# Chairy-neko/TinyRayTracing

Hardware: AMD Instinct MI355X
Metric: Mrays/s (higher is better)
Workload: dtype f32

## Files before the change

tinyraytracing_amd/csrc/trt_api.hip:

```cpp
#include <hip/hip_runtime.h>

#include <dlfcn.h>

#include <algorithm>
#include <cstdio>
#include <cstdlib>
#include <atomic>
#include <limits>
#include <chrono>
#include <cstring>
#include <condition_variable>
#include <memory>
#include <mutex>
#include <string>
#include <thread>
#include <vector>

#include "trt.h"
#include "trt_kernels.h"
#include "trt_wide.h"
#include "trt_oct_build.h"

using namespace trtd;

// ... 50 lines not shown

struct trt_handle {
    int device = 0;
    SceneDev sc{};
    std::vector<void*> scene_allocs;
    std::vector<uint32_t> light_mats;
    std::vector<LightBox> light_boxes;
    uint32_t depth = 0;
    uint32_t bvh2_depth = 0;
    uint32_t shade_tabs = 0;
    uint32_t shade_pad_lds = 0;
    const void* lds_image = nullptr;
    uint32_t lds_image_bytes = 0;
    uint32_t lds_tab[5] = {0, 0, 0, 0, 0};
    int trace_impl = 3;
    int node_kind = 0;
    uint32_t oct_levels = 0;
    bool dbg = false;
    uint32_t rays_per_wave = 256, fill_blocks = 2048, max_blocks = 8192;
    uint32_t traceGrid(uint32_t n) const
    {
        uint32_t b = (n + TRT_TRACE_BLOCK - 1) / TRT_TRACE_BLOCK;
        if (rays_per_wave > 64) {
            const uint32_t want = (uint32_t)(((uint64_t)n + 4ull * rays_per_wave - 1) / (4ull * rays_per_wave));
            b = std::min(b, std::max(fill_blocks, want));
        }
        b = std::min(std::max(b, 8u), std::min(max_blocks, 8192u));
        return (b + 7u) & ~7u;
    }
    uint32_t tail_n = 131072;
// ... 182 lines not shown
        end(stream);
        st.launches[k]++;
    }
};

using ClosestKernel = void (*)(SceneDev, RaySource, f4*, uint32_t, uint32_t*, uint32_t, DeviceStats*, RedoList);
using ShadowKernel = void (*)(SceneDev, ShadowQueue, uint32_t, uint32_t, f4*, uint32_t*, uint32_t, DeviceStats*, uint32_t, RedoList, LightBox);
using FixKernel = void (*)(SceneDev, RaySource, f4*, const f4*, uint32_t, f4*, uint32_t*, uint32_t, RedoList, uint32_t, DeviceStats*);
using ShadeKernel = void (*)(SceneDev, ShadeArgs);
using TailKernel = void (*)(SceneDev, TailArgs);

constexpr uint32_t OCT_LDS_LEVELS = 10;
int traversalOf(const trt_handle* h) { return h->trace_impl == 0 ? 0 : (h->node_kind == 1 ? 1 : (h->depth <= 16 ? 2 : 3)); }
ClosestKernel closestKernel(const trt_handle* h, bool count, int primary)
{
    const ClosestKernel k[4][2][3] = {
        {{k_trace_closest<false, 1, false, 0, 0, 0>, k_trace_closest<false, 1, false, 0, 1, 0>, k_trace_closest<false, 1, false, 0, PRIMARY_LIST, 0>},
         {k_trace_closest<true, 1, false, 0, 0, 0>, k_trace_closest<true, 1, false, 0, 1, 0>, k_trace_closest<true, 1, false, 0, PRIMARY_LIST, 0>}},
        {{k_trace_closest<false, OCT_LDS_LEVELS, true, 3, 0, 1>, k_trace_closest<false, OCT_LDS_LEVELS, true, 3, 1, 1>, k_trace_closest<false, OCT_LDS_LEVELS, true, 3, PRIMARY_LIST, 1>},
         {k_trace_closest<true, OCT_LDS_LEVELS, true, 3, 0, 1>, k_trace_closest<true, OCT_LDS_LEVELS, true, 3, 1, 1>, k_trace_closest<true, OCT_LDS_LEVELS, true, 3, PRIMARY_LIST, 1>}},
        {{k_trace_closest<false, 16, false, 3, 0, 0>, k_trace_closest<false, 16, false, 3, 1, 0>, k_trace_closest<false, 16, false, 3, PRIMARY_LIST, 0>},
         {k_trace_closest<true, 16, false, 3, 0, 0>, k_trace_closest<true, 16, false, 3, 1, 0>, k_trace_closest<true, 16, false, 3, PRIMARY_LIST, 0>}},
        {{k_trace_closest<false, TRT_LDS_STACK_MAX, true, 3, 0, 0>, k_trace_closest<false, TRT_LDS_STACK_MAX, true, 3, 1, 0>, k_trace_closest<false, TRT_LDS_STACK_MAX, true, 3, PRIMARY_LIST, 0>},
         {k_trace_closest<true, TRT_LDS_STACK_MAX, true, 3, 0, 0>, k_trace_closest<true, TRT_LDS_STACK_MAX, true, 3, 1, 0>, k_trace_closest<true, TRT_LDS_STACK_MAX, true, 3, PRIMARY_LIST, 0>}}};
    return k[traversalOf(h)][count][primary];
}
ShadowKernel shadowKernel(const trt_handle* h, bool count)
{
    const ShadowKernel k[4][2] = {{k_trace_shadow<false, 1, false, 0, 0>, k_trace_shadow<true, 1, false, 0, 0>},
                                  {k_trace_shadow<false, OCT_LDS_LEVELS, true, 3, 1>, k_trace_shadow<true, OCT_LDS_LEVELS, true, 3, 1>},
                                  {k_trace_shadow<false, 16, false, 3, 0>, k_trace_shadow<true, 16, false, 3, 0>},
                                  {k_trace_shadow<false, TRT_LDS_STACK_MAX, true, 3, 0>, k_trace_shadow<true, TRT_LDS_STACK_MAX, true, 3, 0>}};
    return k[traversalOf(h)][count];
}
FixKernel fixKernel(const trt_handle* h, bool shadow, int primary)
{
    const FixKernel k[4] = {k_trace_fix<false, 0, 0>, k_trace_fix<false, 1, 0>, k_trace_fix<false, PRIMARY_LIST, 0>, k_trace_fix<true, false, 0>};
    return h->trace_impl == 0 ? nullptr : k[shadow ? 3 : primary];
}
ShadeKernel shadeKernel(uint32_t tabs, int lights, bool list)
{
    const ShadeKernel k[5][2][3] = {
        {{k_shade<31u, SHADE_ONE>, k_shade<31u, SHADE_FEW>, k_shade<31u, SHADE_MANY>}, {k_shade<31u, SHADE_ONE, true>, k_shade<31u, SHADE_FEW, true>, k_shade<31u, SHADE_MANY, true>}},
        {{k_shade<15u, SHADE_ONE>, k_shade<15u, SHADE_FEW>, k_shade<15u, SHADE_MANY>}, {k_shade<15u, SHADE_ONE, true>, k_shade<15u, SHADE_FEW, true>, k_shade<15u, SHADE_MANY, true>}},
        {{k_shade<7u, SHADE_ONE>, k_shade<7u, SHADE_FEW>, k_shade<7u, SHADE_MANY>}, {k_shade<7u, SHADE_ONE, true>, k_shade<7u, SHADE_FEW, true>, k_shade<7u, SHADE_MANY, true>}},
        {{k_shade<3u, SHADE_ONE>, k_shade<3u, SHADE_FEW>, k_shade<3u, SHADE_MANY>}, {k_shade<3u, SHADE_ONE, true>, k_shade<3u, SHADE_FEW, true>, k_shade<3u, SHADE_MANY, true>}},
        {{k_shade<0u, SHADE_ONE>, k_shade<0u, SHADE_FEW>, k_shade<0u, SHADE_MANY>}, {k_shade<0u, SHADE_ONE, true>, k_shade<0u, SHADE_FEW, true>, k_shade<0u, SHADE_MANY, true>}}};
    return k[tabs == 31u ? 0 : (tabs == 15u ? 1 : (tabs == 7u ? 2 : (tabs == 3u ? 3 : 4)))][list][lights];
}
TailKernel tailKernel(bool count, bool list)
{
    if (list) return count ? k_tail<true, 0, true> : k_tail<false, 0, true>;
    return count ? k_tail<true, 0> : k_tail<false, 0>;
}

void launchTraceClosest(const trt_handle* h, ClosestKernel k, FixKernel fix, hipStream_t stream, uint32_t* spill, const RaySource& src, f4* hit, uint32_t n,
// ... 249 lines not shown
        if (total) {
            void* img = nullptr;
            HIPC(hipMalloc(&img, total));
            h->scene_allocs.push_back(img);
            size_t off = 0;
            for (int k = 0; k < 5; ++k)
                if (h->shade_tabs >> k & 1u) {
                    const size_t padded = (h->lds_tab[k] + 15u) & ~15u;
                    HIPC(hipMemcpy((char*)img + off, src[k], padded, hipMemcpyDeviceToDevice));
                    off += padded;
                }
            h->lds_image = img;
            h->lds_image_bytes = (uint32_t)total;
        }
    }

    const uint32_t stack_levels = std::max(h->depth, h->bvh2_depth + 2u);
    uint32_t spill_levels = stack_levels > (uint32_t)TRT_LDS_STACK_MAX ? stack_levels - TRT_LDS_STACK_MAX + 1 : 1;
    if (h->node_kind == 1 && h->oct_levels > OCT_LDS_LEVELS) spill_levels = std::max(spill_levels, 2u * (h->oct_levels - OCT_LDS_LEVELS + 1));
    h->spill_words_per_slot = (size_t)spill_levels * SPILL_STRIDE;
    if (int e = h->spill.ensure(h->spill_words_per_slot * 2 * sizeof(uint32_t))) return e;
    for (hipStream_t& st : h->slot_streams) HIPC(hipStreamCreateWithFlags(&st, hipStreamNonBlocking));
    h->count_rows = countRows(h->sc.n_lights);
    const size_t pinned_words = 2 * (2 * (size_t)h->count_rows + 16);
    HIPC(hipHostMalloc((void**)&h->pinned_counts, pinned_words * sizeof(uint32_t), hipHostMallocDefault));
    std::memset(h->pinned_counts, 0, pinned_words * sizeof(uint32_t));
    if (const char* e = std::getenv("TRT_SLOTS")) h->n_slots = std::atoi(e) >= 2 ? 2 : 1;
    if (const char* e = std::getenv("TRT_TEST_FAIL_AT_BOUNCE")) h->fail_at_bounce = std::atoi(e);
    if (const char* e = std::getenv("TRT_SHADE_PAD_LDS")) {
        h->shade_pad_lds = std::min(100000u, (uint32_t)std::strtoul(e, nullptr, 10));
        for (uint32_t tabs : {31u, 15u, 7u, 3u, 0u})
            for (bool list : {false, true})
                for (int lights : {SHADE_ONE, SHADE_FEW, SHADE_MANY})
                    (void)hipFuncSetAttribute(reinterpret_cast<const void*>(shadeKernel(tabs, lights, list)), hipFuncAttributeMaxDynamicSharedMemorySize, (int)h->shade_pad_lds);
    }

    *out = h.release();
    return TRT_OK;
}
}

extern "C" {

const char* trt_last_error(void) { return g_err.c_str(); }
int trt_abi_version(void) { return TRT_ABI_VERSION; }

int trt_rows_selected(const trt_params* p)
{
    if (!p) return -1;
// ... 241 lines not shown
        SlotLayout::carve(S, (f4*)((char*)h->arena.p + plan.slot_bytes * (size_t)k), plan.N, nl);
        S.redo.count = (uint32_t*)(sb + o_redo) + 2 * k;
        S.d_counts = (uint32_t*)(sb + o_counts + counts_bytes * (size_t)k);
        S.host_counts = h->pinned_counts + (size_t)k * (2 * count_rows + 16);
        S.seq = h->slot_seq[k];
        S.spill = (uint32_t*)h->spill.p + (size_t)k * h->spill_words_per_slot;
    }
    const int lights = nl == 1u ? SHADE_ONE : (nl <= (uint32_t)TRT_MAX_LIGHTS ? SHADE_FEW : SHADE_MANY);
    const uint32_t shade_block = lights == SHADE_ONE ? (uint32_t)TRT_SHADE1_BLOCK : (uint32_t)TRT_SHADEN_BLOCK;
    const uint32_t rows_lds = (in.rows.size() <= shadeRowsLds((int)shade_block) && p->height <= 65536) ? (uint32_t)in.rows.size() : 0u;
    const bool count = (p->flags & TRT_FLAG_COUNT) != 0;
    const int camera = in.list ? PRIMARY_LIST : 1;
    const ClosestKernel camera_k = closestKernel(h, count, camera), queue_k = closestKernel(h, count, 0);
    const FixKernel camera_fix = fixKernel(h, false, camera), queue_fix = fixKernel(h, false, 0), shadow_fix = fixKernel(h, true, 0);
    const ShadowKernel shadow_k = shadowKernel(h, count);
    const ShadeKernel shade_k = shadeKernel(h->shade_tabs, lights, in.list);
    const TailKernel tail_k = tailKernel(count, in.list);
    const ShadeArgs shade_args = shadeArgsOf(h, p, in, d_table, rows_lds, d_stats);
    const TileDesc& td = shade_args.td;
    if (h->dbg)
        std::fprintf(stderr, "%s: k_shade %s, rows in lds %u, grid_ok %u\n", in.list ? "trt_render_pixels" : "trt_render",
                     lights == SHADE_ONE ? "one" : (lights == SHADE_FEW ? "few" : "many"), rows_lds, td.grid_ok);

    Timer tm{h, (p->flags & TRT_FLAG_TIMING) != 0};
    trt_stats st;
    std::memset(&st, 0, sizeof(st));
    hipEvent_t ev_begin = tm.get(0), ev_end = tm.get(1), ev_resolved = tm.get(2);
    if (!ev_begin || !ev_end || !ev_resolved) return fail(TRT_EHIP, "hipEventCreate failed");
    HIPC(hipEventRecord(ev_begin, stream));
    Drain drain{h, slots, plan.slots, stream};
    for (int k = 0; k < plan.slots; ++k) HIPC(hipStreamWaitEvent(slots[k].stream, ev_begin, 0));
// ... 214 lines not shown
    if (int e = checkParams(h, p)) return e;
    if (!out_host) return fail(TRT_EINVAL, "null output buffer");
    return renderTile(h, p, 0u, (uint32_t)p->spp, nullptr, out_host, nullptr, stats, nullptr);
}

int trt_trace_closest(trt_handle* h, uint64_t n, const float* org, const float* dir, float* t, int32_t* tri, float* uv, trt_stats* stats_out)
{
    if (!h || !org || !dir || !t || !tri) return fail(TRT_EINVAL, "trt_trace_closest: null argument");
    if (n == 0) return TRT_OK;
    if (n > 0x7FFF0000ull) return fail(TRT_EINVAL, "ray batch too large");
    HIPC(hipSetDevice(h->device));
    const uint32_t n32 = (uint32_t)n;
    const size_t in_bytes = (size_t)n * 3 * sizeof(float);
    const size_t q16 = (size_t)n * sizeof(f4);
    Layout L;
    const size_t o_ra = L.add(q16, 16), o_rb = L.add(q16, 16), o_hit = L.add(q16, 16), o_org = L.add(in_bytes, 16), o_dir = L.add(in_bytes, 4);
    const size_t o_stats = L.add(sizeof(DeviceStats), 256), o_redo = L.add(2 * sizeof(uint32_t), 64), o_idx = L.add((size_t)n * sizeof(uint32_t), 256);
    if (int e = h->io_buf.ensure(L.bytes)) return e;
    char* b = (char*)h->io_buf.p;
    f4* ra = (f4*)(b + o_ra);
    f4* rb = (f4*)(b + o_rb);
    f4* hit = (f4*)(b + o_hit);
    float* d_org = (float*)(b + o_org);
    float* d_dir = (float*)(b + o_dir);
    DeviceStats* d_stats = (DeviceStats*)(b + o_stats);
    const RedoList redo{(uint32_t*)(b + o_redo), (uint32_t*)(b + o_idx)};
    HIPC(hipMemcpy(d_org, org, in_bytes, hipMemcpyHostToDevice));
    HIPC(hipMemcpy(d_dir, dir, in_bytes, hipMemcpyHostToDevice));
    HIPC(hipMemset(d_stats, 0, o_idx - o_stats));
    hipLaunchKernelGGL(k_pack_rays, dim3(std::min<uint32_t>((n32 + 255) / 256, 65536u)), dim3(256), 0, nullptr, d_org, d_dir, ra, rb, n32);
    Timer tm{h, false};
    hipEvent_t e0 = tm.get(0), e1 = tm.get(1);
    if (!e0 || !e1) return fail(TRT_EHIP, "hipEventCreate failed");
    HIPC(hipEventRecord(e0, nullptr));
    RaySource src{};
    src.ra = ra;
    src.rb = rb;
    launchTraceClosest(h, closestKernel(h, true, 0), fixKernel(h, false, 0), nullptr, (uint32_t*)h->spill.p, src, hit, n32, d_stats, redo);
    HIPC(hipEventRecord(e1, nullptr));
    HIPC(hipDeviceSynchronize());
    HIPC(hipGetLastError());
    float ms = 0.f;
    HIPC(hipEventElapsedTime(&ms, e0, e1));
    std::vector<f4> hh(n);
    HIPC(hipMemcpy(hh.data(), hit, q16, hipMemcpyDeviceToHost));
    for (uint64_t i = 0; i < n; ++i) {
        t[i] = hh[i].x;
        tri[i] = (int32_t)f2u(hh[i].y);
        if (uv) { uv[i * 2] = hh[i].z; uv[i * 2 + 1] = hh[i].w; }
    }
    if (stats_out) {
        DeviceStats ds;
        HIPC(hipMemcpy(&ds, d_stats, sizeof(ds), hipMemcpyDeviceToHost));
        std::memset(stats_out, 0, sizeof(*stats_out));
// ... 298 lines not shown
```

tinyraytracing_amd/csrc/trt_kernels.h:

```cpp
#pragma once
#include <hip/hip_runtime.h>
#include <type_traits>

#include "trt_path.h"
#include "trt_oct.h"

namespace trtd {

#ifndef TRT_TRACE_MINWAVES
#define TRT_TRACE_MINWAVES 0
#endif
#if TRT_TRACE_MINWAVES > 0
#define TRT_TRACE_BOUNDS __launch_bounds__(256, TRT_TRACE_MINWAVES)
#else
#define TRT_TRACE_BOUNDS __launch_bounds__(256)
#endif
constexpr int TRT_TRACE_BLOCK = 256;
#ifndef TRT_LDS_STACK_MAX_LEVELS
#define TRT_LDS_STACK_MAX_LEVELS 16
#endif
constexpr int TRT_LDS_STACK_MAX = TRT_LDS_STACK_MAX_LEVELS;
#ifndef TRT_SHADE1_BLOCK
#define TRT_SHADE1_BLOCK 512
#endif
// ... 112 lines not shown
};
#ifndef TRT_NT
#define TRT_NT 3
#endif
typedef float trt_v4f __attribute__((ext_vector_type(4)));
__device__ __forceinline__ f4 ldNT(const f4* p)
{
    const trt_v4f v = __builtin_nontemporal_load(reinterpret_cast<const trt_v4f*>(p));
    return mk4(v.x, v.y, v.z, v.w);
}
__device__ __forceinline__ void stNT(f4* p, f4 v)
{
    const trt_v4f q = {v.x, v.y, v.z, v.w};
    __builtin_nontemporal_store(q, reinterpret_cast<trt_v4f*>(p));
}
#define TRT_LDQ(bit, ptr) (((TRT_NT) & (bit)) ? ldNT(ptr) : *(ptr))
#define TRT_STQ(bit, ptr, val) do { if ((TRT_NT) & (bit)) stNT((ptr), (val)); else *(ptr) = (val); } while (0)

constexpr int PRIMARY_LIST = 2;
template <int PRIMARY>
__device__ __forceinline__ void fetchRay(const SceneDev& sc, const RaySource& src, uint32_t i, f4& a, f4& b)
{
    if constexpr (PRIMARY == PRIMARY_LIST) primaryRay(sc, src.td, src.s0, i, a, b, PixelList());
    else if (PRIMARY) primaryRay(sc, src.td, src.s0, i, a, b);
    else { a = TRT_LDQ(4, src.ra + i); b = TRT_LDQ(4, src.rb + i); }
}

struct RedoList {
    uint32_t* count;
    uint32_t* idx;
};

constexpr uint32_t TRT_REF_IDLE = 0xFFFFFFFFu;
constexpr uint32_t TRT_REF_DONE = 0xFFFFFFFEu;

struct TraceProbe {
    uint32_t n_inner = 0, n_tri = 0;
    uint32_t wave_inner = 0, wave_tri = 0;
    uint32_t c_in = 0, c_lf = 0, c_done = 0, c_it = 0;
};

template <bool SHADOW>
__device__ __forceinline__ void storeResult(const SceneDev& sc, f3 o, f3 d, float best_t, int32_t best_tri, uint32_t best_flags, uint32_t idx, uint32_t pid,
                                            f4* __restrict__ hit, const f4* __restrict__ sw, uint32_t light_mat, f4* __restrict__ Lacc, bool any)
{
    if (!SHADOW) {
        float u = 0.f, v = 0.f;
        if (best_tri >= 0) {
            float t, un, vn, det;
            if (triTest(sc.tri_isect[best_tri], o, d, t, un, vn, det)) { u = un / det; v = vn / det; }
        }
        TRT_STQ(8, hit + idx, mk4(best_t, u2f((uint32_t)best_tri), u, v));
    } else if (any ? best_tri < 0 : (best_tri >= 0 && (best_flags >> 8) == light_mat)) {
        const f4 w = TRT_LDQ(16, sw + idx);
        f4 L = TRT_LDQ(32, Lacc + pid);
        L.x = L.x + w.x; L.y = L.y + w.y; L.z = L.z + w.z;
        TRT_STQ(32, Lacc + pid, L);
    }
}

template <bool SHADOW, bool OCT = false>
// ... 18 lines not shown
        const bool vis = any ? best_tri < 0 : (best_tri >= 0 && (best_flags >> 8) == light_mat);
        f4 w = mk4(0, 0, 0, 0), L = w;
        if (vis) { w = TRT_LDQ(16, sw + idx); L = TRT_LDQ(32, Lacc + pid); }
        float e;
        const bool pass = boxTest(ba.x, ba.y, ba.z, ba.w, bb.x, bb.y, o, inv, e);
        if (special || (best_tri >= 0 && ((OCT && !pass) || best_t < trt_leaf_floor(e, sc.leaf_alpha)))) return true;
        if (vis) {
            L.x = L.x + w.x; L.y = L.y + w.y; L.z = L.z + w.z;
            TRT_STQ(32, Lacc + pid, L);
        }
    }
    return false;
}

constexpr int TRT_PEND_SLOTS = 4;
template <bool COUNT, int STRIDE, bool GLM>
__device__ __forceinline__ void uniformWalkImpl(const SceneDev& sc, f3 o, f3 d, f3 inv, bool valid, bool special, f4* __restrict__ my_pend, float& best_t, int32_t& best_tri,
                                                uint32_t& best_flags, uint32_t& n_inner, uint32_t& n_tri)
{
    const uint32_t n_nodes = sc.n_nodes;
    uint32_t reach = valid ? 1u : 0u;
    uint32_t n_pend = 0;
    auto flush = [&]() {
        for (uint32_t s = 0; ballotb(s < n_pend) != 0ull; ++s) {
            if (s < n_pend) {
                const f4 e = my_pend[s * STRIDE];
                const float t = e.x / e.y;
                if (!(t < TRT_T_MIN) && !(t < e.w)) {
                    const uint32_t pk = f2u(e.z);
                    const int32_t j = (int32_t)(pk & 0xFFu);
                    const uint32_t fl = f2u(sc.tri_isect[j].c.z);
                    bool take = t < best_t;
                    if (t == best_t && best_tri >= 0) {
                        const bool em = (fl & 1u) != 0, bem = (best_flags & 1u) != 0;
                        const uint32_t first = (pk >> 8) & 0xFFu, cnt = pk >> 16;
                        const bool same_leaf = (uint32_t)best_tri >= first && (uint32_t)best_tri < first + cnt;
                        take = same_leaf ? em : (em ? (!bem || j < best_tri) : (!bem && j > best_tri));
                    }
                    if (take) { best_t = t; best_tri = j; best_flags = fl; }
                }
            }
        }
        n_pend = 0;
    };
    for (uint32_t ni = 0; ni < n_nodes; ++ni) {
        const bool at = (reach >> ni) & 1u;
// ... 37 lines not shown
            }
        }
    }
    flush();
}
template <bool COUNT, int STRIDE = TRT_TRACE_BLOCK>
__device__ __forceinline__ void uniformWalk(const SceneDev& sc, f3 o, f3 d, bool valid, f4* __restrict__ my_pend, float& best_t, int32_t& best_tri,
                                            uint32_t& best_flags, uint32_t& n_inner, uint32_t& n_tri)
{
    const f3 inv = mk3(1.0f / d.x, 1.0f / d.y, 1.0f / d.z);
    const bool special = valid && raySpecial(inv);
    if (ballotb(special) != 0ull) uniformWalkImpl<COUNT, STRIDE, true>(sc, o, d, inv, valid, special, my_pend, best_t, best_tri, best_flags, n_inner, n_tri);
    else uniformWalkImpl<COUNT, STRIDE, false>(sc, o, d, inv, valid, false, my_pend, best_t, best_tri, best_flags, n_inner, n_tri);
}

template <bool SHADOW, bool COUNT, int PRIMARY>
__device__ __forceinline__ void traceQueueUniform(const SceneDev& sc, const RaySource& src, uint32_t n, f4* __restrict__ hit,
                                                  const f4* __restrict__ sw, uint32_t light_mat, f4* __restrict__ Lacc, DeviceStats* stats, bool any_flag,
                                                  f4* __restrict__ pend)
{
    const bool any = SHADOW && any_flag;
    uint32_t n_inner = 0, n_tri = 0;
    const uint32_t lb = xcdSwizzle(blockIdx.x, gridDim.x);
    const uint32_t stride = gridDim.x * TRT_TRACE_BLOCK;
    f4* my_pend = pend + threadIdx.x;
    __shared__ uint32_t s_parked[2 * TRT_TRACE_BLOCK];
    uint32_t* my_parked = s_parked + (threadIdx.x >> 6) * 128u;
    const uint32_t lane = threadIdx.x & 63u;
    uint32_t n_parked = 0;
    auto rewalk = [&]() {
        for (uint32_t base = 0; base < n_parked; base += 64u) {
            const bool valid = base + lane < n_parked;
            const uint32_t i = my_parked[valid ? base + lane : 0u];
            f4 a, b;
            fetchRay<PRIMARY>(sc, src, i, a, b);
            const f3 o = mk3(a.x, a.y, a.z), d = mk3(a.w, b.x, b.y);
            float best_t = any ? b.w : TRT_INF;
            int32_t best_tri = -1;
            uint32_t best_flags = 0u;
            uint32_t ni = 0, nt = 0;
            uniformWalkImpl<false, TRT_TRACE_BLOCK, true>(sc, o, d, mk3(1.0f / d.x, 1.0f / d.y, 1.0f / d.z), valid, valid, my_pend, best_t, best_tri, best_flags, ni, nt);
            if (valid) storeResult<SHADOW>(sc, o, d, best_t, best_tri, best_flags, i, SHADOW ? f2u(b.z) : 0u, hit, sw, light_mat, Lacc, any);
        }
        if (lane == 0 && n_parked) atomicAdd(&stats->redo_rays, n_parked);
        n_parked = 0;
    };
    for (uint32_t base = lb * TRT_TRACE_BLOCK; base < n; base += stride) {
        const uint32_t i = base + threadIdx.x;
        const bool valid = i < n;
        const uint32_t ii = valid ? i : n - 1;
        f4 a, b;
        fetchRay<PRIMARY>(sc, src, ii, a, b);
        const f3 o = mk3(a.x, a.y, a.z), d = mk3(a.w, b.x, b.y);
        const f3 inv = mk3(1.0f / d.x, 1.0f / d.y, 1.0f / d.z);
        float best_t = any ? b.w : TRT_INF;
        int32_t best_tri = -1;
        uint32_t best_flags = 0u;
        uniformWalkImpl<COUNT, TRT_TRACE_BLOCK, false>(sc, o, d, inv, valid, false, my_pend, best_t, best_tri, best_flags, n_inner, n_tri);
        const bool special = valid && raySpecial(inv);
        if (valid && !special) storeResult<SHADOW>(sc, o, d, best_t, best_tri, best_flags, i, SHADOW ? f2u(b.z) : 0u, hit, sw, light_mat, Lacc, any);
        const unsigned long long m_sp = ballotb(special);
        if (m_sp != 0ull) {
            const uint32_t at = n_parked + (uint32_t)__popcll(m_sp & ((1ull << lane) - 1ull));
            if (special && at < 128u) my_parked[at] = i;
            n_parked += (uint32_t)__popcll(m_sp);
        }
    }
    if (n_parked != 0u && n_parked <= 128u) rewalk();
    else if (n_parked > 128u) {
        for (uint32_t base = lb * TRT_TRACE_BLOCK; base < n; base += stride) {
            const uint32_t i = base + threadIdx.x;
            const bool valid = i < n;
            f4 a, b;
            fetchRay<PRIMARY>(sc, src, valid ? i : n - 1, a, b);
            const f3 o = mk3(a.x, a.y, a.z), d = mk3(a.w, b.x, b.y);
            const f3 inv = mk3(1.0f / d.x, 1.0f / d.y, 1.0f / d.z);
            const bool special = valid && raySpecial(inv);
            if (ballotb(special) == 0ull) continue;
            float best_t = any ? b.w : TRT_INF;
            int32_t best_tri = -1;
            uint32_t best_flags = 0u;
            uint32_t ni = 0, nt = 0;
            uniformWalkImpl<false, TRT_TRACE_BLOCK, true>(sc, o, d, inv, special, special, my_pend, best_t, best_tri, best_flags, ni, nt);
            if (special) storeResult<SHADOW>(sc, o, d, best_t, best_tri, best_flags, i, SHADOW ? f2u(b.z) : 0u, hit, sw, light_mat, Lacc, any);
        }
        if (lane == 0) atomicAdd(&stats->redo_rays, n_parked);
    }
    if (COUNT) {
        const unsigned long long si = waveSum(n_inner), st = waveSum(n_tri);
        if ((threadIdx.x & 63) == 0) {
            atomicAdd(&stats->inner_visits[SHADOW ? 1 : 0], si);
            atomicAdd(&stats->tri_tests[SHADOW ? 1 : 0], st);
        }
    }
}


template <bool SHADOW, bool COUNT, int DEPTH, bool SPILL, int IMPL, int PRIMARY, int NK>
__device__ __forceinline__ void traceQueuePersistent(const SceneDev& sc, const RaySource& src, uint32_t n, f4* __restrict__ hit,
// ... 232 lines not shown
    if (COUNT) {
        const unsigned long long si = waveSum(pr.n_inner), st = waveSum(pr.n_tri), wi = waveSum(pr.wave_inner), wt = waveSum(pr.wave_tri);
        if (lane == 0) {
            atomicAdd(&stats->inner_visits[SHADOW ? 1 : 0], si);
            atomicAdd(&stats->tri_tests[SHADOW ? 1 : 0], st);
            atomicAdd(&stats->wave_inner_steps, wi);
            atomicAdd(&stats->wave_leaf_steps, wt);
            atomicAdd(&stats->census_inner, (unsigned long long)pr.c_in);
            atomicAdd(&stats->census_leaf, (unsigned long long)pr.c_lf);
            atomicAdd(&stats->census_done, (unsigned long long)pr.c_done);
            atomicAdd(&stats->census_iters, (unsigned long long)pr.c_it);
        }
    }
}

template <bool SHADOW, bool COUNT, int DEPTH, bool SPILL, int IMPL, int PRIMARY, int NK>
__device__ __forceinline__ void traceQueue(const SceneDev& sc, const RaySource& src, uint32_t n, f4* __restrict__ hit,
                                           const f4* __restrict__ sw, uint32_t light_mat, f4* __restrict__ Lacc, uint32_t* __restrict__ spill,
                                           uint32_t spill_stride, DeviceStats* stats, uint32_t* smem, bool any_flag, RedoList redo, const LightBox& lbox)
{
    if constexpr (IMPL == 0) traceQueueUniform<SHADOW, COUNT, PRIMARY>(sc, src, n, hit, sw, light_mat, Lacc, stats, any_flag, reinterpret_cast<f4*>(smem));
    else if constexpr (NK == 1) traceQueuePersistentOct<SHADOW, COUNT, DEPTH, SPILL, PRIMARY>(sc, src, n, hit, sw, light_mat, Lacc, spill, spill_stride, stats, smem, any_flag, redo, lbox);
    else traceQueuePersistent<SHADOW, COUNT, DEPTH, SPILL, IMPL, PRIMARY, NK>(sc, src, n, hit, sw, light_mat, Lacc, spill, spill_stride, stats, smem, any_flag, redo);
}

template <bool COUNT, int DEPTH, bool SPILL, int IMPL, int PRIMARY, int NK>
__global__ TRT_TRACE_BOUNDS void k_trace_closest(SceneDev sc, RaySource src, f4* __restrict__ hit, uint32_t n,
                                                 uint32_t* __restrict__ spill, uint32_t spill_stride, DeviceStats* stats, RedoList redo)
{
    __shared__ __attribute__((aligned(16))) uint32_t smem[IMPL == 0 ? TRT_PEND_SLOTS * 4 * TRT_TRACE_BLOCK : (NK == 1 ? 2 : 1) * DEPTH * TRT_TRACE_BLOCK];
    const LightBox nobox = {{0.f, 0.f, 0.f}, {0.f, 0.f, 0.f}};
    traceQueue<false, COUNT, DEPTH, SPILL, IMPL, PRIMARY, NK>(sc, src, n, hit, nullptr, 0u, nullptr, spill, spill_stride, stats, smem, false, redo, nobox);
}

template <bool COUNT, int DEPTH, bool SPILL, int IMPL, int NK>
__global__ TRT_TRACE_BOUNDS void k_trace_shadow(SceneDev sc, ShadowQueue sq, uint32_t n, uint32_t light_mat, f4* __restrict__ Lacc,
                                                uint32_t* __restrict__ spill, uint32_t spill_stride, DeviceStats* stats, uint32_t any, RedoList redo, LightBox lbox)
{
    __shared__ __attribute__((aligned(16))) uint32_t smem[IMPL == 0 ? TRT_PEND_SLOTS * 4 * TRT_TRACE_BLOCK : (NK == 1 ? 2 : 1) * DEPTH * TRT_TRACE_BLOCK];
    RaySource src;
    src.ra = sq.sa;
    src.rb = sq.sb;
    src.s0 = 0;
    traceQueue<true, COUNT, DEPTH, SPILL, IMPL, false, NK>(sc, src, n, nullptr, sq.sw, light_mat, Lacc, spill, spill_stride, stats, smem, any != 0u, redo, lbox);
}

constexpr uint32_t TRT_FIX_BLOCKS = 32;
template <bool SHADOW, int PRIMARY, int NK>
__global__ __launch_bounds__(TRT_TRACE_BLOCK) void k_trace_fix(SceneDev sc, RaySource src, f4* __restrict__ hit, const f4* __restrict__ sw, uint32_t light_mat,
                                                               f4* __restrict__ Lacc, uint32_t* __restrict__ spill, uint32_t spill_stride, RedoList redo, uint32_t any_flag,
                                                               DeviceStats* stats)
{
    __shared__ __attribute__((aligned(16))) uint32_t smem[TRT_LDS_STACK_MAX * TRT_TRACE_BLOCK];
    const uint32_t n = *redo.count;
    if (n == 0u) return;
    {
        LdsStack<TRT_LDS_STACK_MAX, true> stk;
        stk.lds = smem + threadIdx.x;
        stk.spill = spill + (size_t)blockIdx.x * TRT_TRACE_BLOCK + threadIdx.x;
// ... 114 lines not shown
    __device__ int operator()(const TileDesc& td, uint32_t r) const
    {
        int y = 0;
        if (in_lds) {
            y = lds[r];
#if defined(__HIP_DEVICE_COMPILE__)
            asm volatile("" : "+v"(y));
#endif
        } else {
            y = td.rows[r];
        }
        return y;
    }
};

template <int LIGHTS>
__device__ inline ShadowQueue shadeQueue(const ShadeArgs& A, uint32_t li)
{
    if (LIGHTS == SHADE_MANY) return A.sq_arena.queue(li);
    return A.sq[li];
}
template <uint32_t TABS, int LIGHTS, bool LIST = false, int BLOCK = (LIGHTS == SHADE_ONE ? TRT_SHADE1_BLOCK : TRT_SHADEN_BLOCK),
          int WAVES = (LIGHTS == SHADE_ONE ? TRT_SHADE1_WAVES : TRT_SHADEN_WAVES)>
__global__ __launch_bounds__(BLOCK, WAVES) void k_shade(SceneDev sc, ShadeArgs A)
{
    constexpr int TRT_SHADE_BLOCK = BLOCK;
    constexpr uint32_t TRT_SHADE_ROWS_LDS = shadeRowsLds(BLOCK);
    __shared__ uint32_t s_cnt[3 * (TRT_SHADE_BLOCK / 64 + 1)];
    __shared__ uint32_t s_cnt2[2 * (2 * (TRT_SHADE_BLOCK / 64) + 2)];
    __shared__ uint32_t s_shaded, s_depth;
    __shared__ __attribute__((aligned(16))) uint32_t s_tab[TABS ? TRT_SHADE_LDS_TABLE_BYTES / 4 : 4];
    __shared__ uint16_t s_rows[LIST ? 1 : TRT_SHADE_ROWS_LDS];
    if (threadIdx.x == 0) { s_shaded = 0; s_depth = 0; }
    if (!LIST)
        for (uint32_t r = threadIdx.x; r < A.rows_lds; r += TRT_SHADE_BLOCK) s_rows[r] = (uint16_t)A.td.rows[r];
    std::conditional_t<LIST, PixelList, RowsShade> rows;
    if constexpr (!LIST) {
        rows.lds = s_rows;
        rows.in_lds = A.rows_lds != 0u;
    }
    bool rows_visible = A.rows_lds == 0u;
    {
        uint32_t off = 0;
        auto at = [&](uint32_t bytes) -> const void* { const void* q = s_tab + off / 4; off += (bytes + 15u) & ~15u; return q; };
        if (TABS & 1u) sc.materials = static_cast<const MaterialDev*>(at(A.lds_mat_bytes));
        if (TABS & 2u) sc.lights = static_cast<const LightDev*>(at(A.lds_light_bytes));
        if (TABS & 4u) sc.light_cum = static_cast<const float*>(at(A.lds_cum_bytes));
        if (TABS & 8u) sc.light_tris = static_cast<const LightTriDev*>(at(A.lds_ltri_bytes));
        if (TABS & 16u) sc.tri_shade = static_cast<const TriShade*>(at(A.lds_tshade_bytes));
    }
    bool staged = TABS == 0u;
    int parity = 0, parity2 = 0;
    uint32_t bounce_depth = 0;
    const uint32_t per_grid = gridDim.x * TRT_SHADE_BLOCK;
    auto loadTile = [&](uint32_t i, f4& hit4, f4& ra, f4& rb, f4& bt) {
        hit4 = mk4(TRT_INF, u2f(0xFFFFFFFFu), 0.0f, 0.0f); ra = mk4(0, 0, 0, 0); rb = ra; bt = mk4(1.0f, 1.0f, 1.0f, 0.0f);
        if (i < A.n) {
            hit4 = TRT_LDQ(1, A.hit + i);
            if (!A.primary) { ra = TRT_LDQ(1, A.qin.ra + i); rb = TRT_LDQ(1, A.qin.rb + i); bt = TRT_LDQ(1, A.qin.bt + i); }
        }
    };
#if TRT_SHADE_PIPE
    f4 n_hit, n_ra, n_rb, n_bt;
    loadTile(blockIdx.x * TRT_SHADE_BLOCK + threadIdx.x, n_hit, n_ra, n_rb, n_bt);
#endif
    for (uint32_t base = blockIdx.x * TRT_SHADE_BLOCK; base < A.n; base += per_grid) {
        const uint32_t i = base + threadIdx.x;
        f4 hit4, ra, rb, bt;
#if TRT_SHADE_PIPE
        hit4 = n_hit; ra = n_ra; rb = n_rb; bt = n_bt;
#else
        loadTile(i, hit4, ra, rb, bt);
#endif
        if (!staged || !rows_visible) {
            if (!staged) {
                f4* l = reinterpret_cast<f4*>(s_tab);
                for (uint32_t w = threadIdx.x; w < A.lds_image_words; w += TRT_SHADE_BLOCK) l[w] = A.lds_image[w];
            }
            __syncthreads();
            staged = true;
            rows_visible = true;
        }
#if defined(__HIP_DEVICE_COMPILE__)
        asm volatile("" : "+v"(hit4.x), "+v"(ra.x), "+v"(rb.x), "+v"(bt.x));
#endif
#if TRT_SHADE_PIPE
        loadTile(i + per_grid, n_hit, n_ra, n_rb, n_bt);
#endif
        ShadeCtx c;
        c.had_hit = c.shade_ok = c.add_L = false;
        if (i < A.n) {
            if (A.primary) {
                primaryRay(sc, A.td, A.s0, i, ra, rb, rows);
                shadeBegin(sc, A.td, A.s0, ra, rb, bt, hit4, c, rows);
                A.Lacc[i] = c.add_L ? mk4(0.0f + c.addL.x, 0.0f + c.addL.y, 0.0f + c.addL.z, 0.0f) : mk4(0.0f, 0.0f, 0.0f, 0.0f);
            } else {
                shadeBegin(sc, A.td, A.s0, ra, rb, bt, hit4, c, rows);
                if (c.add_L) {
                    f4 L = A.Lacc[c.pid];
                    L.x = L.x + c.addL.x; L.y = L.y + c.addL.y; L.z = L.z + c.addL.z;
                    A.Lacc[c.pid] = L;
                }
            }
            if (c.had_hit) bounce_depth = c.depth + 1u > bounce_depth ? c.depth + 1u : bounce_depth;
        }
        const unsigned long long ok_ballot = ballotb(c.shade_ok);
        if ((threadIdx.x & 63u) == 0 && ok_ballot) atomicAdd(&s_shaded, (uint32_t)__popcll(ok_ballot));

        uint32_t pend_base = 0;
        const uint32_t* pend_s = nullptr;
        bool pend_emit = false;
// ... 217 lines not shown
{
    for (uint32_t t = threadIdx.x; t < 2u * n; t += blockDim.x) {
        const uint32_t c = t >> 1, which = t & 1u;
        uint32_t v = counts[(size_t)c * stride + b + which];
        if (c == 0u && which == 1u) v = (uint32_t)pair[0];
        if (n > 1u && c == n - 1u && which == 0u) v = (uint32_t)(pair[0] >> 32);
        out[t] = v;
    }
    __threadfence_system();
    __syncthreads();
    if (threadIdx.x == 0) {
        __hip_atomic_store(const_cast<uint32_t*>(out) + seq_word, seq, __ATOMIC_RELEASE, __HIP_MEMORY_SCOPE_SYSTEM);
    }
}

__global__ __launch_bounds__(256) void k_pack_rays(const float* __restrict__ org, const float* __restrict__ dir, f4* __restrict__ ra, f4* __restrict__ rb, uint32_t n)
{
    const uint32_t stride = gridDim.x * blockDim.x;
    for (uint32_t i = blockIdx.x * blockDim.x + threadIdx.x; i < n; i += stride) {
        ra[i] = mk4(org[(size_t)i * 3], org[(size_t)i * 3 + 1], org[(size_t)i * 3 + 2], dir[(size_t)i * 3]);
        rb[i] = mk4(dir[(size_t)i * 3 + 1], dir[(size_t)i * 3 + 2], u2f(i), 0.0f);
    }
}

}
```

Measured before the change: 23160.

## Store 8-byte hit records and recompute barycentrics in shade for tiny scenes

For scenes with at most 64 triangles on the wave-uniform walk, the closest-hit kernel writes only (t, tri) as 8-byte records instead of 16-byte ones. The shade kernel stages the triangle intersection data in LDS and recomputes u,v from the ray, and a separate kernel rebuilds full hit records for the trace-only API path. Shadow and closest walks also read triangle flags from an LDS copy instead of global memory. This cuts hit-buffer traffic and global flag loads, at the cost of extra LDS use and duplicated triangle tests in shading.

```diff
diff --git a/tinyraytracing_amd/csrc/trt_api.hip b/tinyraytracing_amd/csrc/trt_api.hip
--- a/tinyraytracing_amd/csrc/trt_api.hip
+++ b/tinyraytracing_amd/csrc/trt_api.hip
@@ -88,6 +88,8 @@
     uint32_t lds_image_bytes = 0;
     uint32_t lds_tab[5] = {0, 0, 0, 0, 0};
     int trace_impl = 3;
+    bool slim_walk = false;
+    bool hit8 = false;
     int node_kind = 0;
     uint32_t oct_levels = 0;
     bool dbg = false;
@@ -300,6 +302,12 @@
 int traversalOf(const trt_handle* h) { return h->trace_impl == 0 ? 0 : (h->node_kind == 1 ? 1 : (h->depth <= 16 ? 2 : 3)); }
 ClosestKernel closestKernel(const trt_handle* h, bool count, int primary)
 {
+    if (h->trace_impl == 0 && h->hit8) {
+        const ClosestKernel s[2][3] = {
+            {k_trace_closest<false, 1, false, 0, 0, 0, true, true>, k_trace_closest<false, 1, false, 0, 1, 0, true, true>, k_trace_closest<false, 1, false, 0, PRIMARY_LIST, 0, true, true>},
+            {k_trace_closest<true, 1, false, 0, 0, 0, true, true>, k_trace_closest<true, 1, false, 0, 1, 0, true, true>, k_trace_closest<true, 1, false, 0, PRIMARY_LIST, 0, true, true>}};
+        return s[count][primary];
+    }
     const ClosestKernel k[4][2][3] = {
         {{k_trace_closest<false, 1, false, 0, 0, 0>, k_trace_closest<false, 1, false, 0, 1, 0>, k_trace_closest<false, 1, false, 0, PRIMARY_LIST, 0>},
          {k_trace_closest<true, 1, false, 0, 0, 0>, k_trace_closest<true, 1, false, 0, 1, 0>, k_trace_closest<true, 1, false, 0, PRIMARY_LIST, 0>}},
@@ -313,6 +321,7 @@
 }
 ShadowKernel shadowKernel(const trt_handle* h, bool count)
 {
+    if (h->trace_impl == 0 && h->slim_walk) return count ? k_trace_shadow<true, 1, false, 0, 0, true> : k_trace_shadow<false, 1, false, 0, 0, true>;
     const ShadowKernel k[4][2] = {{k_trace_shadow<false, 1, false, 0, 0>, k_trace_shadow<true, 1, false, 0, 0>},
                                   {k_trace_shadow<false, OCT_LDS_LEVELS, true, 3, 1>, k_trace_shadow<true, OCT_LDS_LEVELS, true, 3, 1>},
                                   {k_trace_shadow<false, 16, false, 3, 0>, k_trace_shadow<true, 16, false, 3, 0>},
@@ -324,8 +333,16 @@
     const FixKernel k[4] = {k_trace_fix<false, 0, 0>, k_trace_fix<false, 1, 0>, k_trace_fix<false, PRIMARY_LIST, 0>, k_trace_fix<true, false, 0>};
     return h->trace_impl == 0 ? nullptr : k[shadow ? 3 : primary];
 }
-ShadeKernel shadeKernel(uint32_t tabs, int lights, bool list)
-{
+ShadeKernel shadeKernel(uint32_t tabs, int lights, bool list, bool hit8)
+{
+    if (hit8) {
+        const ShadeKernel s[2][3] = {
+            {k_shade<31u, SHADE_ONE, false, TRT_SHADE1_BLOCK, TRT_SHADE1_WAVES, true>, k_shade<31u, SHADE_FEW, false, TRT_SHADEN_BLOCK, TRT_SHADEN_WAVES, true>,
+             k_shade<31u, SHADE_MANY, false, TRT_SHADEN_BLOCK, TRT_SHADEN_WAVES, true>},
+            {k_shade<31u, SHADE_ONE, true, TRT_SHADE1_BLOCK, TRT_SHADE1_WAVES, true>, k_shade<31u, SHADE_FEW, true, TRT_SHADEN_BLOCK, TRT_SHADEN_WAVES, true>,
+             k_shade<31u, SHADE_MANY, true, TRT_SHADEN_BLOCK, TRT_SHADEN_WAVES, true>}};
+        return s[list][lights];
+    }
     const ShadeKernel k[5][2][3] = {
         {{k_shade<31u, SHADE_ONE>, k_shade<31u, SHADE_FEW>, k_shade<31u, SHADE_MANY>}, {k_shade<31u, SHADE_ONE, true>, k_shade<31u, SHADE_FEW, true>, k_shade<31u, SHADE_MANY, true>}},
         {{k_shade<15u, SHADE_ONE>, k_shade<15u, SHADE_FEW>, k_shade<15u, SHADE_MANY>}, {k_shade<15u, SHADE_ONE, true>, k_shade<15u, SHADE_FEW, true>, k_shade<15u, SHADE_MANY, true>}},
@@ -605,6 +622,10 @@
             h->lds_image_bytes = (uint32_t)total;
         }
     }
+    h->slim_walk = h->trace_impl == 0 && s->n_tris <= 64;
+    if (const char* e = std::getenv("TRT_SLIM_WALK")) h->slim_walk = h->slim_walk && std::atoi(e) != 0;
+    h->hit8 = h->slim_walk && h->shade_tabs == 31u;
+    if (im.dbg) std::fprintf(stderr, "trt_create: slim walk %d, 8-byte hit records %d\n", (int)h->slim_walk, (int)h->hit8);
 
     const uint32_t stack_levels = std::max(h->depth, h->bvh2_depth + 2u);
     uint32_t spill_levels = stack_levels > (uint32_t)TRT_LDS_STACK_MAX ? stack_levels - TRT_LDS_STACK_MAX + 1 : 1;
@@ -623,7 +644,9 @@
         for (uint32_t tabs : {31u, 15u, 7u, 3u, 0u})
             for (bool list : {false, true})
                 for (int lights : {SHADE_ONE, SHADE_FEW, SHADE_MANY})
-                    (void)hipFuncSetAttribute(reinterpret_cast<const void*>(shadeKernel(tabs, lights, list)), hipFuncAttributeMaxDynamicSharedMemorySize, (int)h->shade_pad_lds);
+                    for (bool hit8 : {false, true})
+                        if (!hit8 || tabs == 31u)
+                            (void)hipFuncSetAttribute(reinterpret_cast<const void*>(shadeKernel(tabs, lights, list, hit8)), hipFuncAttributeMaxDynamicSharedMemorySize, (int)h->shade_pad_lds);
     }
 
     *out = h.release();
@@ -895,7 +918,7 @@
     const ClosestKernel camera_k = closestKernel(h, count, camera), queue_k = closestKernel(h, count, 0);
     const FixKernel camera_fix = fixKernel(h, false, camera), queue_fix = fixKernel(h, false, 0), shadow_fix = fixKernel(h, true, 0);
     const ShadowKernel shadow_k = shadowKernel(h, count);
-    const ShadeKernel shade_k = shadeKernel(h->shade_tabs, lights, in.list);
+    const ShadeKernel shade_k = shadeKernel(h->shade_tabs, lights, in.list, h->hit8);
     const TailKernel tail_k = tailKernel(count, in.list);
     const ShadeArgs shade_args = shadeArgsOf(h, p, in, d_table, rows_lds, d_stats);
     const TileDesc& td = shade_args.td;
@@ -1140,7 +1163,7 @@
     const size_t in_bytes = (size_t)n * 3 * sizeof(float);
     const size_t q16 = (size_t)n * sizeof(f4);
     Layout L;
-    const size_t o_ra = L.add(q16, 16), o_rb = L.add(q16, 16), o_hit = L.add(q16, 16), o_org = L.add(in_bytes, 16), o_dir = L.add(in_bytes, 4);
+    const size_t o_ra = L.add(q16, 16), o_rb = L.add(q16, 16), o_hit = L.add(q16, 16), o_hit8 = L.add(h->hit8 ? q16 / 2 : 0, 16), o_org = L.add(in_bytes, 16), o_dir = L.add(in_bytes, 4);
     const size_t o_stats = L.add(sizeof(DeviceStats), 256), o_redo = L.add(2 * sizeof(uint32_t), 64), o_idx = L.add((size_t)n * sizeof(uint32_t), 256);
     if (int e = h->io_buf.ensure(L.bytes)) return e;
     char* b = (char*)h->io_buf.p;
@@ -1162,8 +1185,10 @@
     RaySource src{};
     src.ra = ra;
     src.rb = rb;
-    launchTraceClosest(h, closestKernel(h, true, 0), fixKernel(h, false, 0), nullptr, (uint32_t*)h->spill.p, src, hit, n32, d_stats, redo);
+    f4* hit8 = (f4*)(b + o_hit8);
+    launchTraceClosest(h, closestKernel(h, true, 0), fixKernel(h, false, 0), nullptr, (uint32_t*)h->spill.p, src, h->hit8 ? hit8 : hit, n32, d_stats, redo);
     HIPC(hipEventRecord(e1, nullptr));
+    if (h->hit8) hipLaunchKernelGGL(k_hit_uv, dim3(std::min<uint32_t>((n32 + 255) / 256, 65536u)), dim3(256), 0, nullptr, h->sc, (const f4*)ra, (const f4*)rb, (const f4*)hit8, hit, n32);
     HIPC(hipDeviceSynchronize());
     HIPC(hipGetLastError());
     float ms = 0.f;
diff --git a/tinyraytracing_amd/csrc/trt_kernels.h b/tinyraytracing_amd/csrc/trt_kernels.h
--- a/tinyraytracing_amd/csrc/trt_kernels.h
+++ b/tinyraytracing_amd/csrc/trt_kernels.h
@@ -150,8 +150,12 @@
     const trt_v4f q = {v.x, v.y, v.z, v.w};
     __builtin_nontemporal_store(q, reinterpret_cast<trt_v4f*>(p));
 }
+typedef float trt_v2f __attribute__((ext_vector_type(2)));
+__device__ __forceinline__ trt_v2f ldNT2(const trt_v2f* p) { return __builtin_nontemporal_load(p); }
 #define TRT_LDQ(bit, ptr) (((TRT_NT) & (bit)) ? ldNT(ptr) : *(ptr))
+#define TRT_LDQ2(bit, ptr) (((TRT_NT) & (bit)) ? ldNT2(ptr) : *(ptr))
 #define TRT_STQ(bit, ptr, val) do { if ((TRT_NT) & (bit)) stNT((ptr), (val)); else *(ptr) = (val); } while (0)
+#define TRT_STQ2(bit, ptr, val) do { if ((TRT_NT) & (bit)) __builtin_nontemporal_store((val), (ptr)); else *(ptr) = (val); } while (0)
 
 constexpr int PRIMARY_LIST = 2;
 template <int PRIMARY>
@@ -176,11 +180,14 @@
     uint32_t c_in = 0, c_lf = 0, c_done = 0, c_it = 0;
 };
 
-template <bool SHADOW>
+template <bool SHADOW, bool HIT8 = false>
 __device__ __forceinline__ void storeResult(const SceneDev& sc, f3 o, f3 d, float best_t, int32_t best_tri, uint32_t best_flags, uint32_t idx, uint32_t pid,
                                             f4* __restrict__ hit, const f4* __restrict__ sw, uint32_t light_mat, f4* __restrict__ Lacc, bool any)
 {
-    if (!SHADOW) {
+    if (!SHADOW && HIT8) {
+        const trt_v2f r = {best_t, u2f((uint32_t)best_tri)};
+        TRT_STQ2(8, reinterpret_cast<trt_v2f*>(hit) + idx, r);
+    } else if (!SHADOW) {
         float u = 0.f, v = 0.f;
         if (best_tri >= 0) {
             float t, un, vn, det;
@@ -229,9 +236,9 @@
 }
 
 constexpr int TRT_PEND_SLOTS = 4;
-template <bool COUNT, int STRIDE, bool GLM>
+template <bool COUNT, int STRIDE, bool GLM, bool FLAGS_LDS = false>
 __device__ __forceinline__ void uniformWalkImpl(const SceneDev& sc, f3 o, f3 d, f3 inv, bool valid, bool special, f4* __restrict__ my_pend, float& best_t, int32_t& best_tri,
-                                                uint32_t& best_flags, uint32_t& n_inner, uint32_t& n_tri)
+                                                uint32_t& best_flags, uint32_t& n_inner, uint32_t& n_tri, const uint32_t* tri_flags = nullptr)
 {
     const uint32_t n_nodes = sc.n_nodes;
     uint32_t reach = valid ? 1u : 0u;
@@ -244,7 +251,7 @@
                 if (!(t < TRT_T_MIN) && !(t < e.w)) {
                     const uint32_t pk = f2u(e.z);
                     const int32_t j = (int32_t)(pk & 0xFFu);
-                    const uint32_t fl = f2u(sc.tri_isect[j].c.z);
+                    const uint32_t fl = FLAGS_LDS ? tri_flags[j] : f2u(sc.tri_isect[j].c.z);
                     bool take = t < best_t;
                     if (t == best_t && best_tri >= 0) {
                         const bool em = (fl & 1u) != 0, bem = (best_flags & 1u) != 0;
@@ -312,7 +319,7 @@
     else uniformWalkImpl<COUNT, STRIDE, false>(sc, o, d, inv, valid, false, my_pend, best_t, best_tri, best_flags, n_inner, n_tri);
 }
 
-template <bool SHADOW, bool COUNT, int PRIMARY>
+template <bool SHADOW, bool COUNT, int PRIMARY, bool HIT8 = false, bool PIPE = false>
 __device__ __forceinline__ void traceQueueUniform(const SceneDev& sc, const RaySource& src, uint32_t n, f4* __restrict__ hit,
                                                   const f4* __restrict__ sw, uint32_t light_mat, f4* __restrict__ Lacc, DeviceStats* stats, bool any_flag,
                                                   f4* __restrict__ pend)
@@ -322,6 +329,11 @@
     const uint32_t lb = xcdSwizzle(blockIdx.x, gridDim.x);
     const uint32_t stride = gridDim.x * TRT_TRACE_BLOCK;
     f4* my_pend = pend + threadIdx.x;
+    __shared__ uint32_t s_flags[PIPE ? 64 : 1];
+    if (PIPE) {
+        if (threadIdx.x < (sc.n_tris < 64u ? sc.n_tris : 64u)) s_flags[threadIdx.x] = f2u(sc.tri_isect[threadIdx.x].c.z);
+        __syncthreads();
+    }
     __shared__ uint32_t s_parked[2 * TRT_TRACE_BLOCK];
     uint32_t* my_parked = s_parked + (threadIdx.x >> 6) * 128u;
     const uint32_t lane = threadIdx.x & 63u;
@@ -337,8 +349,8 @@
             int32_t best_tri = -1;
             uint32_t best_flags = 0u;
             uint32_t ni = 0, nt = 0;
-            uniformWalkImpl<false, TRT_TRACE_BLOCK, true>(sc, o, d, mk3(1.0f / d.x, 1.0f / d.y, 1.0f / d.z), valid, valid, my_pend, best_t, best_tri, best_flags, ni, nt);
-            if (valid) storeResult<SHADOW>(sc, o, d, best_t, best_tri, best_flags, i, SHADOW ? f2u(b.z) : 0u, hit, sw, light_mat, Lacc, any);
+            uniformWalkImpl<false, TRT_TRACE_BLOCK, true, PIPE>(sc, o, d, mk3(1.0f / d.x, 1.0f / d.y, 1.0f / d.z), valid, valid, my_pend, best_t, best_tri, best_flags, ni, nt, s_flags);
+            if (valid) storeResult<SHADOW, HIT8>(sc, o, d, best_t, best_tri, best_flags, i, SHADOW ? f2u(b.z) : 0u, hit, sw, light_mat, Lacc, any);
         }
         if (lane == 0 && n_parked) atomicAdd(&stats->redo_rays, n_parked);
         n_parked = 0;
@@ -354,9 +366,9 @@
         float best_t = any ? b.w : TRT_INF;
         int32_t best_tri = -1;
         uint32_t best_flags = 0u;
-        uniformWalkImpl<COUNT, TRT_TRACE_BLOCK, false>(sc, o, d, inv, valid, false, my_pend, best_t, best_tri, best_flags, n_inner, n_tri);
+        uniformWalkImpl<COUNT, TRT_TRACE_BLOCK, false, PIPE>(sc, o, d, inv, valid, false, my_pend, best_t, best_tri, best_flags, n_inner, n_tri, s_flags);
         const bool special = valid && raySpecial(inv);
-        if (valid && !special) storeResult<SHADOW>(sc, o, d, best_t, best_tri, best_flags, i, SHADOW ? f2u(b.z) : 0u, hit, sw, light_mat, Lacc, any);
+        if (valid && !special) storeResult<SHADOW, HIT8>(sc, o, d, best_t, best_tri, best_flags, i, SHADOW ? f2u(b.z) : 0u, hit, sw, light_mat, Lacc, any);
         const unsigned long long m_sp = ballotb(special);
         if (m_sp != 0ull) {
             const uint32_t at = n_parked + (uint32_t)__popcll(m_sp & ((1ull << lane) - 1ull));
@@ -379,8 +391,8 @@
             int32_t best_tri = -1;
             uint32_t best_flags = 0u;
             uint32_t ni = 0, nt = 0;
-            uniformWalkImpl<false, TRT_TRACE_BLOCK, true>(sc, o, d, inv, special, special, my_pend, best_t, best_tri, best_flags, ni, nt);
-            if (special) storeResult<SHADOW>(sc, o, d, best_t, best_tri, best_flags, i, SHADOW ? f2u(b.z) : 0u, hit, sw, light_mat, Lacc, any);
+            uniformWalkImpl<false, TRT_TRACE_BLOCK, true, PIPE>(sc, o, d, inv, special, special, my_pend, best_t, best_tri, best_flags, ni, nt, s_flags);
+            if (special) storeResult<SHADOW, HIT8>(sc, o, d, best_t, best_tri, best_flags, i, SHADOW ? f2u(b.z) : 0u, hit, sw, light_mat, Lacc, any);
         }
         if (lane == 0) atomicAdd(&stats->redo_rays, n_parked);
     }
@@ -643,26 +655,27 @@
     }
 }
 
-template <bool SHADOW, bool COUNT, int DEPTH, bool SPILL, int IMPL, int PRIMARY, int NK>
+template <bool SHADOW, bool COUNT, int DEPTH, bool SPILL, int IMPL, int PRIMARY, int NK, bool HIT8 = false, bool PIPE = false>
 __device__ __forceinline__ void traceQueue(const SceneDev& sc, const RaySource& src, uint32_t n, f4* __restrict__ hit,
                                            const f4* __restrict__ sw, uint32_t light_mat, f4* __restrict__ Lacc, uint32_t* __restrict__ spill,
                                            uint32_t spill_stride, DeviceStats* stats, uint32_t* smem, bool any_flag, RedoList redo, const LightBox& lbox)
 {
-    if constexpr (IMPL == 0) traceQueueUniform<SHADOW, COUNT, PRIMARY>(sc, src, n, hit, sw, light_mat, Lacc, stats, any_flag, reinterpret_cast<f4*>(smem));
+    static_assert(IMPL == 0 || !(HIT8 || PIPE), "8-byte hit records and the flags in LDS belong to the wave-uniform walk");
+    if constexpr (IMPL == 0) traceQueueUniform<SHADOW, COUNT, PRIMARY, HIT8, PIPE>(sc, src, n, hit, sw, light_mat, Lacc, stats, any_flag, reinterpret_cast<f4*>(smem));
     else if constexpr (NK == 1) traceQueuePersistentOct<SHADOW, COUNT, DEPTH, SPILL, PRIMARY>(sc, src, n, hit, sw, light_mat, Lacc, spill, spill_stride, stats, smem, any_flag, redo, lbox);
     else traceQueuePersistent<SHADOW, COUNT, DEPTH, SPILL, IMPL, PRIMARY, NK>(sc, src, n, hit, sw, light_mat, Lacc, spill, spill_stride, stats, smem, any_flag, redo);
 }
 
-template <bool COUNT, int DEPTH, bool SPILL, int IMPL, int PRIMARY, int NK>
+template <bool COUNT, int DEPTH, bool SPILL, int IMPL, int PRIMARY, int NK, bool HIT8 = false, bool PIPE = false>
 __global__ TRT_TRACE_BOUNDS void k_trace_closest(SceneDev sc, RaySource src, f4* __restrict__ hit, uint32_t n,
                                                  uint32_t* __restrict__ spill, uint32_t spill_stride, DeviceStats* stats, RedoList redo)
 {
     __shared__ __attribute__((aligned(16))) uint32_t smem[IMPL == 0 ? TRT_PEND_SLOTS * 4 * TRT_TRACE_BLOCK : (NK == 1 ? 2 : 1) * DEPTH * TRT_TRACE_BLOCK];
     const LightBox nobox = {{0.f, 0.f, 0.f}, {0.f, 0.f, 0.f}};
-    traceQueue<false, COUNT, DEPTH, SPILL, IMPL, PRIMARY, NK>(sc, src, n, hit, nullptr, 0u, nullptr, spill, spill_stride, stats, smem, false, redo, nobox);
-}
-
-template <bool COUNT, int DEPTH, bool SPILL, int IMPL, int NK>
+    traceQueue<false, COUNT, DEPTH, SPILL, IMPL, PRIMARY, NK, HIT8, PIPE>(sc, src, n, hit, nullptr, 0u, nullptr, spill, spill_stride, stats, smem, false, redo, nobox);
+}
+
+template <bool COUNT, int DEPTH, bool SPILL, int IMPL, int NK, bool PIPE = false>
 __global__ TRT_TRACE_BOUNDS void k_trace_shadow(SceneDev sc, ShadowQueue sq, uint32_t n, uint32_t light_mat, f4* __restrict__ Lacc,
                                                 uint32_t* __restrict__ spill, uint32_t spill_stride, DeviceStats* stats, uint32_t any, RedoList redo, LightBox lbox)
 {
@@ -671,7 +684,7 @@
     src.ra = sq.sa;
     src.rb = sq.sb;
     src.s0 = 0;
-    traceQueue<true, COUNT, DEPTH, SPILL, IMPL, false, NK>(sc, src, n, nullptr, sq.sw, light_mat, Lacc, spill, spill_stride, stats, smem, any != 0u, redo, lbox);
+    traceQueue<true, COUNT, DEPTH, SPILL, IMPL, false, NK, false, PIPE>(sc, src, n, nullptr, sq.sw, light_mat, Lacc, spill, spill_stride, stats, smem, any != 0u, redo, lbox);
 }
 
 constexpr uint32_t TRT_FIX_BLOCKS = 32;
@@ -816,6 +829,17 @@
     }
 };
 
+__device__ __forceinline__ void hitBarycentrics(const TriIsect* isect, const f4& ra, const f4& rb, f4& hit4)
+{
+    const int32_t tri = (int32_t)f2u(hit4.y);
+    float u = 0.f, v = 0.f;
+    if (tri >= 0) {
+        float t, un, vn, det;
+        if (triTest(isect[tri], mk3(ra.x, ra.y, ra.z), mk3(ra.w, rb.x, rb.y), t, un, vn, det)) { u = un / det; v = vn / det; }
+    }
+    hit4.z = u;
+    hit4.w = v;
+}
 template <int LIGHTS>
 __device__ inline ShadowQueue shadeQueue(const ShadeArgs& A, uint32_t li)
 {
@@ -823,7 +847,7 @@
     return A.sq[li];
 }
 template <uint32_t TABS, int LIGHTS, bool LIST = false, int BLOCK = (LIGHTS == SHADE_ONE ? TRT_SHADE1_BLOCK : TRT_SHADEN_BLOCK),
-          int WAVES = (LIGHTS == SHADE_ONE ? TRT_SHADE1_WAVES : TRT_SHADEN_WAVES)>
+          int WAVES = (LIGHTS == SHADE_ONE ? TRT_SHADE1_WAVES : TRT_SHADEN_WAVES), bool HIT8 = false>
 __global__ __launch_bounds__(BLOCK, WAVES) void k_shade(SceneDev sc, ShadeArgs A)
 {
     constexpr int TRT_SHADE_BLOCK = BLOCK;
@@ -833,6 +857,8 @@
     __shared__ uint32_t s_shaded, s_depth;
     __shared__ __attribute__((aligned(16))) uint32_t s_tab[TABS ? TRT_SHADE_LDS_TABLE_BYTES / 4 : 4];
     __shared__ uint16_t s_rows[LIST ? 1 : TRT_SHADE_ROWS_LDS];
+    __shared__ __attribute__((aligned(16))) uint32_t s_isect[HIT8 ? 64 * 12 : 4];
+    const TriIsect* isect = reinterpret_cast<const TriIsect*>(s_isect);
     if (threadIdx.x == 0) { s_shaded = 0; s_depth = 0; }
     if (!LIST)
         for (uint32_t r = threadIdx.x; r < A.rows_lds; r += TRT_SHADE_BLOCK) s_rows[r] = (uint16_t)A.td.rows[r];
@@ -851,14 +877,19 @@
         if (TABS & 8u) sc.light_tris = static_cast<const LightTriDev*>(at(A.lds_ltri_bytes));
         if (TABS & 16u) sc.tri_shade = static_cast<const TriShade*>(at(A.lds_tshade_bytes));
     }
-    bool staged = TABS == 0u;
+    bool staged = TABS == 0u && !HIT8;
     int parity = 0, parity2 = 0;
     uint32_t bounce_depth = 0;
     const uint32_t per_grid = gridDim.x * TRT_SHADE_BLOCK;
     auto loadTile = [&](uint32_t i, f4& hit4, f4& ra, f4& rb, f4& bt) {
         hit4 = mk4(TRT_INF, u2f(0xFFFFFFFFu), 0.0f, 0.0f); ra = mk4(0, 0, 0, 0); rb = ra; bt = mk4(1.0f, 1.0f, 1.0f, 0.0f);
         if (i < A.n) {
-            hit4 = TRT_LDQ(1, A.hit + i);
+            if (HIT8) {
+                const trt_v2f h = TRT_LDQ2(1, reinterpret_cast<const trt_v2f*>(A.hit) + i);
+                hit4.x = h.x; hit4.y = h.y;
+            } else {
+                hit4 = TRT_LDQ(1, A.hit + i);
+            }
             if (!A.primary) { ra = TRT_LDQ(1, A.qin.ra + i); rb = TRT_LDQ(1, A.qin.rb + i); bt = TRT_LDQ(1, A.qin.bt + i); }
         }
     };
@@ -877,7 +908,13 @@
         if (!staged || !rows_visible) {
             if (!staged) {
                 f4* l = reinterpret_cast<f4*>(s_tab);
-                for (uint32_t w = threadIdx.x; w < A.lds_image_words; w += TRT_SHADE_BLOCK) l[w] = A.lds_image[w];
+                if (TABS)
+                    for (uint32_t w = threadIdx.x; w < A.lds_image_words; w += TRT_SHADE_BLOCK) l[w] = A.lds_image[w];
+                if (HIT8) {
+                    f4* li = reinterpret_cast<f4*>(s_isect);
+                    const uint32_t words = 3u * (sc.n_tris < 64u ? sc.n_tris : 64u);
+                    for (uint32_t w = threadIdx.x; w < words; w += TRT_SHADE_BLOCK) li[w] = reinterpret_cast<const f4*>(sc.tri_isect)[w];
+                }
             }
             __syncthreads();
             staged = true;
@@ -894,9 +931,11 @@
         if (i < A.n) {
             if (A.primary) {
                 primaryRay(sc, A.td, A.s0, i, ra, rb, rows);
+                if (HIT8) hitBarycentrics(isect, ra, rb, hit4);
                 shadeBegin(sc, A.td, A.s0, ra, rb, bt, hit4, c, rows);
                 A.Lacc[i] = c.add_L ? mk4(0.0f + c.addL.x, 0.0f + c.addL.y, 0.0f + c.addL.z, 0.0f) : mk4(0.0f, 0.0f, 0.0f, 0.0f);
             } else {
+                if (HIT8) hitBarycentrics(isect, ra, rb, hit4);
                 shadeBegin(sc, A.td, A.s0, ra, rb, bt, hit4, c, rows);
                 if (c.add_L) {
                     f4 L = A.Lacc[c.pid];
@@ -1144,6 +1183,17 @@
     }
 }
 
+__global__ __launch_bounds__(256) void k_hit_uv(SceneDev sc, const f4* __restrict__ ra, const f4* __restrict__ rb, const f4* __restrict__ hit8, f4* __restrict__ out, uint32_t n)
+{
+    const uint32_t stride = gridDim.x * blockDim.x;
+    for (uint32_t i = blockIdx.x * blockDim.x + threadIdx.x; i < n; i += stride) {
+        const trt_v2f h = reinterpret_cast<const trt_v2f*>(hit8)[i];
+        f4 hit4 = mk4(h.x, h.y, 0.0f, 0.0f);
+        hitBarycentrics(sc.tri_isect, ra[i], rb[i], hit4);
+        out[i] = hit4;
+    }
+}
+
 __global__ __launch_bounds__(256) void k_pack_rays(const float* __restrict__ org, const float* __restrict__ dir, f4* __restrict__ ra, f4* __restrict__ rb, uint32_t n)
 {
     const uint32_t stride = gridDim.x * blockDim.x;
```

Measured after the change: 23680, median of 6. +2.3%, better.
